# itshawi/data-accelerator

Measured on AMD Instinct MI355X. Metric: events/sec (node) + p99 latency, SimulatedData IoT Flow, higher is better.
Workload: dtype fp64/int64 columns (no reduced precision)

## Files before the change

### dxa/ops/csrc/json_parse.hip

```cpp
#include "dxa_common.h"
#include <type_traits>
#include "decimal_dd.h"
#include "dxa_ts.h"

namespace {

enum : int32_t {
  FT_STRUCT = 0, FT_BOOL = 1, FT_LONG = 2, FT_DOUBLE = 3, FT_STRING = 4, FT_RAW = 5,
  FT_TIMESTAMP = 6, FT_INT = 7, FT_DATE = 8, FT_DECIMAL = 9,
  FT_SKIP = 10,
};

struct ParseArgs {
  uint8_t* buf;
  const int64_t* offs;
  int64_t n;
  const uint64_t* lut_keys;
  const int32_t* lut_node;
  int32_t lut_cap;
  const int32_t* node_type;
  const int32_t* val_slot;
  const int32_t* len_slot;
  int32_t nnodes;
  int64_t* vals;
  int32_t* lens;
  uint8_t* valid;
  uint8_t* row_ok;
  const int32_t* first_child;
  const int32_t* next_sib;
  const int32_t* key_word;
  const int32_t* key_len;
  const uint64_t* key_words;
  int32_t nkey_words;
  const int64_t* ends;
  int64_t* vals2;
  int32_t* lens2;
  uint8_t* valid2;
  int32_t nkv, nkl, nkn;
  const int32_t* zslots;
  int32_t nz;
};

#define G1 __attribute__((address_space(1)))
typedef G1 uint8_t gu8;
struct GArgs {
  gu8* buf;
  const G1 int64_t* offs;
  int64_t n;
  const G1 uint64_t* lut_keys;
  const G1 int32_t* lut_node;
  int32_t lut_cap;
  const G1 int32_t* node_type;
  const G1 int32_t* val_slot;
  const G1 int32_t* len_slot;
  int32_t nnodes;
  G1 int64_t* vals;
  G1 int32_t* lens;
  gu8* valid;
  gu8* row_ok;
  const G1 int32_t* first_child;
  const G1 int32_t* next_sib;
  const G1 int32_t* key_word;
  const G1 int32_t* key_len;
  const G1 uint64_t* key_words;
  int32_t nkey_words;
  const G1 int64_t* ends;
  G1 int64_t* vals2;
  G1 int32_t* lens2;
  gu8* valid2;
  int32_t nkv, nkl, nkn;
  const G1 int32_t* zslots;
  int32_t nz;
  __device__ __forceinline__ G1 int64_t* vrow(int v) const {
    return v < nkv ? vals + (int64_t)v * n : vals2 + (int64_t)(v - nkv) * n;
  }
  __device__ __forceinline__ G1 int32_t* lrow(int l) const {
    return l < nkl ? lens + (int64_t)l * n : lens2 + (int64_t)(l - nkl) * n;
  }
  __device__ __forceinline__ gu8* drow(int k) const {
    return k < nkn ? valid + (int64_t)k * n : valid2 + (int64_t)(k - nkn) * n;
  }
};

__device__ __forceinline__ GArgs to_global(const ParseArgs& p) {
  GArgs g;
  g.buf = (gu8*)p.buf;
  g.offs = (const G1 int64_t*)p.offs;
  g.n = p.n;
  g.lut_keys = (const G1 uint64_t*)p.lut_keys;
  g.lut_node = (const G1 int32_t*)p.lut_node;
  g.lut_cap = p.lut_cap;
  g.node_type = (const G1 int32_t*)p.node_type;
  g.val_slot = (const G1 int32_t*)p.val_slot;
  g.len_slot = (const G1 int32_t*)p.len_slot;
  g.nnodes = p.nnodes;
  g.vals = (G1 int64_t*)p.vals;
  g.lens = (G1 int32_t*)p.lens;
  g.valid = (gu8*)p.valid;
  g.row_ok = (gu8*)p.row_ok;
  g.first_child = (const G1 int32_t*)p.first_child;
  g.next_sib = (const G1 int32_t*)p.next_sib;
  g.key_word = (const G1 int32_t*)p.key_word;
  g.key_len = (const G1 int32_t*)p.key_len;
  g.key_words = (const G1 uint64_t*)p.key_words;
  g.nkey_words = p.nkey_words;
  g.ends = (const G1 int64_t*)p.ends;
  g.vals2 = (G1 int64_t*)p.vals2;
  g.lens2 = (G1 int32_t*)p.lens2;
  g.valid2 = (gu8*)p.valid2;
  g.nkv = p.nkv;
  g.nkl = p.nkl;
  g.nkn = p.nkn;
  g.zslots = (const G1 int32_t*)p.zslots;
  g.nz = p.nz;
  return g;
}

__constant__ uint64_t kPow10i[9] = {1ull, 10ull, 100ull, 1000ull, 10000ull, 100000ull, 1000000ull, 10000000ull,
                                    100000000ull};
__constant__ double kPow10[23] = {1e0,  1e1,  1e2,  1e3,  1e4,  1e5,  1e6,  1e7,  1e8,  1e9,  1e10, 1e11,
                                  1e12, 1e13, 1e14, 1e15, 1e16, 1e17, 1e18, 1e19, 1e20, 1e21, 1e22};


#define G3 __attribute__((address_space(3)))
template <bool LDS>
struct Tables {
  typedef typename std::conditional<LDS, const G3 int32_t*, const G1 int32_t*>::type I32P;
  typedef typename std::conditional<LDS, const G3 uint64_t*, const G1 uint64_t*>::type U64P;
  I32P node_type, val_slot, len_slot, first_child, next_sib, key_word, key_len, lut_node;
  U64P key_words, lut_keys;
  int32_t lut_cap;
};

__host__ __device__ inline int64_t tables_lds_bytes(int32_t nnodes, int32_t nkw, int32_t lut_cap) {
  return (int64_t)nkw * 8 + (int64_t)lut_cap * 8 + (int64_t)(8 * nnodes + lut_cap) * 4;
}

template <bool LDS>
__device__ __forceinline__ Tables<LDS> load_tables(const GArgs& a);

template <>
__device__ __forceinline__ Tables<false> load_tables<false>(const GArgs& a) {
  Tables<false> t;
  t.node_type = a.node_type; t.val_slot = a.val_slot; t.len_slot = a.len_slot;
  t.first_child = a.first_child; t.next_sib = a.next_sib; t.key_word = a.key_word; t.key_len = a.key_len;
  t.lut_node = a.lut_node; t.key_words = a.key_words; t.lut_keys = a.lut_keys; t.lut_cap = a.lut_cap;
  return t;
}

extern __shared__ uint64_t dyn_lds[];

template <>
__device__ __forceinline__ Tables<true> load_tables<true>(const GArgs& a) {
  G3 uint64_t* u64 = (G3 uint64_t*)dyn_lds;
  G3 uint64_t* kw = u64;
  G3 uint64_t* lk = u64 + a.nkey_words;
  G3 int32_t* i32 = (G3 int32_t*)(lk + a.lut_cap);
  const int nn = a.nnodes;
  G3 int32_t* arr[7] = {i32, i32 + nn, i32 + 2 * nn, i32 + 3 * nn, i32 + 4 * nn, i32 + 5 * nn, i32 + 6 * nn};
  G3 int32_t* ln = i32 + 8 * nn;
  for (int i = threadIdx.x; i < a.nkey_words; i += blockDim.x) kw[i] = a.key_words[i];
  for (int i = threadIdx.x; i < a.lut_cap; i += blockDim.x) { lk[i] = a.lut_keys[i]; ln[i] = a.lut_node[i]; }
  for (int i = threadIdx.x; i < nn; i += blockDim.x) {
    arr[0][i] = a.node_type[i]; arr[1][i] = a.val_slot[i]; arr[2][i] = a.len_slot[i];
    arr[3][i] = a.first_child[i]; arr[4][i] = a.next_sib[i]; arr[5][i] = a.key_word[i]; arr[6][i] = a.key_len[i];
  }
  __syncthreads();
// ... 539 lines not shown
  } b{rd};
  auto num = [&](int64_t& i, int digits, int& v) -> bool {
    v = 0;
    for (int k = 0; k < digits; ++k) {
      if (i >= e || !is_digit(b[i])) return false;
      v = v * 10 + (b[i] - '0');
      ++i;
    }
    return true;
  };
  int64_t i = s;
  int y, mo, d, hh = 0, mi = 0, ss = 0;
  if (!num(i, 4, y) || i >= e || b[i] != '-') return false;
  ++i;
  if (!num(i, 2, mo) || i >= e || b[i] != '-') return false;
  ++i;
  if (!num(i, 2, d)) return false;
  int64_t frac_us = 0;
  int64_t tz_us = 0;
  if (i < e && (b[i] == 'T' || b[i] == ' ')) {
    ++i;
    if (!num(i, 2, hh) || i >= e || b[i] != ':') return false;
    ++i;
    if (!num(i, 2, mi)) return false;
    if (i < e && b[i] == ':') { ++i; if (!num(i, 2, ss)) return false; }
    if (i < e && b[i] == '.') {
      ++i;
      int64_t scale = 100000;
      while (i < e && is_digit(b[i])) { frac_us += (b[i] - '0') * scale; scale /= 10; ++i; }
    }
    if (i < e && b[i] == 'Z') ++i;
    else if (i < e && (b[i] == '+' || b[i] == '-')) {
      const bool neg = b[i] == '-';
      ++i;
      int th, tm = 0;
      if (!num(i, 2, th)) return false;
      if (i < e && b[i] == ':') ++i;
      if (i < e) { if (!num(i, 2, tm)) return false; }
      tz_us = ((int64_t)th * 3600 + tm * 60) * 1000000ll;
      if (neg) tz_us = -tz_us;
    }
  } else if (!date_only_ok) {
    return false;
  }
  if (i != e) return false;
  if (mo < 1 || mo > 12 || d < 1 || d > 31 || hh > 23 || mi > 59 || ss > 60) return false;
  const int64_t days = dxa::days_from_civil(y, (unsigned)mo, (unsigned)d);
  out = ((days * 86400 + hh * 3600 + mi * 60 + ss) * 1000000ll) + frac_us - tz_us;
  return true;
}

constexpr uint32_t kTopUp = 32;
typedef int16_t StackT;
template <bool LDS>
__global__ __launch_bounds__(256) __attribute__((amdgpu_waves_per_eu(5))) void json_parse_kernel(ParseArgs pa) {
  const GArgs a = to_global(pa);
  const Tables<LDS> tb = load_tables<LDS>(a);
  const int64_t row = (int64_t)blockIdx.x * blockDim.x + threadIdx.x;
  if (row >= a.n) return;
  for (int j = 0; j < a.nz; ++j) {
    a.vrow(a.zslots[2 * j])[row] = 0;
    a.lrow(a.zslots[2 * j + 1])[row] = 0;
  }
  const int64_t n = a.n;
  Reader r;
  r.buf = a.buf;
  r.p = a.offs[row];
  r.end = a.ends ? a.ends[row] : a.offs[row + 1];
  r.wb = -256;
  r.lim = a.offs[n] + 16;
  __shared__ uint32_t s_win[17][256];
  r.win = (G3U32*)&s_win[0][threadIdx.x];

  __shared__ StackT s_stack[kMaxDepth][256];
  __shared__ StackT s_expect[kMaxDepth][256];
  StackT* stack_ = &s_stack[0][threadIdx.x];
  StackT* expect_ = &s_expect[0][threadIdx.x];
#define stack(i) stack_[(i) * 256]
#define expect(i) expect_[(i) * 256]
  int depth = 0;
  bool ok = false;
  bool comma = false;
  int store_node = -1;
  __shared__ uint64_t s_seen[256];
  s_seen[threadIdx.x] = 0;

  if (r.ws_cur() != '{') goto done;
  ++r.p;
  stack(0) = 0;
  expect(0) = tb.first_child[0];
  depth = 1;
  a.drow(0)[row] = 1;
  uint32_t nextc;
  while (true) {
    r.top_up(kTopUp);
    nextc = 256u;
    uint32_t c;
    int node;
    if (comma) {
      const int ex = expect(depth - 1);
      uint32_t nx = 256u;
      if (ex >= 0 && quote_key_colon(r, r.p, r.end, tb.key_words + tb.key_word[ex], tb.key_len[ex], nx)) {
        comma = false;
        store_node = -1;
        node = ex;
        expect(depth - 1) = tb.next_sib[node];
        c = (nx == 256u || nx == ' ' || nx == '\n' || nx == '\r' || nx == '\t') ? r.ws_cur() : nx;
        goto have_value;
      }
    }
    c = r.ws_cur();
    if (c == '}') {
// ... 135 lines not shown
      }
      if (c == 't' || c == 'f') {
        const int64_t s = r.p;
        const bool v = (c == 't');
        if (!take_literal(r, c)) break;
        if (t == FT_BOOL) {
          a.vrow(vs)[row] = v ? 1 : 0;
          a.drow(node)[row] = 1;
        } else if (t == FT_STRING) {
          a.vrow(vs)[row] = s;
          a.lrow(ls)[row] = v ? 4 : 5;
          a.drow(node)[row] = 1;
        }
        goto after_value;
      }
      if (c == 'n') {
        if (!take_literal(r, c)) break;
        goto after_value;
      }
      break;
    }
  skip_any: {
      const int64_t s0 = r.p;
      if (c == '-' || is_digit(c)) {
        if (!skip_number(r, c, nextc)) break;
      } else if (c == '"') {
        int64_t s, e;
        bool esc;
        if (!scan_string(r, s, e, esc, nextc)) break;
      } else if (!skip_value(r)) {
        break;
      }
      if (store_node >= 0) {
        a.vrow(tb.val_slot[store_node])[row] = s0;
        a.lrow(tb.len_slot[store_node])[row] = (int32_t)(r.p - s0);
        a.drow(store_node)[row] = 1;
      }
    }
  after_value:
    c = (nextc == 256u || nextc == ' ' || nextc == '\n' || nextc == '\r' || nextc == '\t') ? r.ws_cur() : nextc;
    if (c == ',') { ++r.p; comma = true; continue; }
    if (c == '}') continue;
    break;
  }
  if (ok) {
    r.skip_ws();
    ok = r.p >= r.end;
  }
done:
  a.row_ok[row] = ok ? 1 : 0;
  if (!ok) {
    for (int k = 0; k < a.nnodes; ++k) a.drow(k)[row] = 0;
  }
#undef stack
#undef expect
}

__global__ __launch_bounds__(256) void null_count_kernel(const uint8_t* __restrict__ valid, int64_t n,
                                                         unsigned long long* __restrict__ nulls) {
  const int k = blockIdx.y;
  const int64_t r0 = ((int64_t)blockIdx.x * blockDim.x + threadIdx.x) * 8;
  unsigned long long cnt = 0;
  if (r0 < n) {
    const int32_t avail = n - r0 < 8 ? (int32_t)(n - r0) : 8;
    const uint8_t* p = valid + (int64_t)k * n + r0;
    const uintptr_t x = reinterpret_cast<uintptr_t>(p);
    const int m = (int)(x & 7);
    const uint64_t* q = reinterpret_cast<const uint64_t*>(x - m);
    uint64_t v = q[0] >> (8 * m);
    if (m && 8 - m < avail) v |= q[1] << (64 - 8 * m);
    if (avail < 8) v &= (1ull << (8 * avail)) - 1;
    cnt = (unsigned long long)(avail - __popcll(v & 0x0101010101010101ull));
  }
#pragma unroll
  for (int o = 32; o >= 1; o >>= 1) cnt += __shfl_xor(cnt, o);
  if ((threadIdx.x & 63) == 0 && cnt) atomicAdd(&nulls[k], cnt);
}

__device__ __forceinline__ uint64_t nl_bytes(uint64_t x) {
  const uint64_t t = x ^ 0x0a0a0a0a0a0a0a0aull;
  const uint64_t y = ((t & 0x7f7f7f7f7f7f7f7full) + 0x7f7f7f7f7f7f7f7full) | t;
  return ~y & 0x8080808080808080ull;
}

__device__ __forceinline__ void nl_masks(const uint8_t* buf, int64_t p, int64_t end, uint64_t& m0, uint64_t& m1) {
  m0 = m1 = 0;
  if (p >= end) return;
  const uint4 v = *reinterpret_cast<const uint4*>(buf + p);
  m0 = nl_bytes(((uint64_t)v.y << 32) | v.x);
  m1 = nl_bytes(((uint64_t)v.w << 32) | v.z);
  const int64_t rem = end - p;
  if (rem < 16) {
    if (rem <= 8) { m1 = 0; if (rem < 8) m0 &= (1ull << (8 * rem)) - 1; }
    else m1 &= (1ull << (8 * (rem - 8))) - 1;
  }
}

__device__ __forceinline__ uint32_t nl_pack8(uint64_t m) { return (uint32_t)(((m >> 7) * 0x0102040810204080ull) >> 56); }

__global__ __launch_bounds__(256) void count_newlines_kernel(const uint8_t* __restrict__ buf, int64_t len,
                                                             int64_t seg, int64_t nseg,
                                                             int64_t* __restrict__ counts,
                                                             uint16_t* __restrict__ bits) {
  const int lane = threadIdx.x & 63;
  const int64_t s = (int64_t)blockIdx.x * 4 + (threadIdx.x >> 6);
  if (s >= nseg) return;
  const int64_t beg = s * seg;
  const int64_t end = beg + seg < len ? beg + seg : len;
// ... 14 lines not shown
                                                                  int64_t* __restrict__ pos, int64_t cap,
                                                                  int64_t delta) {
  const int lane = threadIdx.x & 63;
  const int64_t s = (int64_t)blockIdx.x * 4 + (threadIdx.x >> 6);
  if (s >= nseg) return;
  const int64_t beg = s * seg;
  const int64_t end = beg + seg < len ? beg + seg : len;
  int64_t k = base[s];
  for (int64_t it = beg; it < end; it += 1024) {
    const int64_t p = it + lane * 16;
    uint32_t m = p < end ? bits[p >> 4] : 0u;
    const uint32_t c = __popc(m);
    uint32_t incl = c;
    for (int o = 1; o < 64; o <<= 1) {
      const uint32_t v = __shfl_up(incl, o, 64);
      if (lane >= o) incl += v;
    }
    int64_t q = k + (incl - c);
    while (m) { const int j = __builtin_ctz(m); if (q < cap) pos[q] = p + j + delta; ++q; m &= m - 1; }
    k += __shfl(incl, 63, 64);
  }
}

__global__ void zero_bytes_kernel(uint8_t* __restrict__ p, int64_t nbytes) {
  const uintptr_t a = reinterpret_cast<uintptr_t>(p);
  const int64_t head = (int64_t)((16 - (a & 15)) & 15) < nbytes ? (int64_t)((16 - (a & 15)) & 15) : nbytes;
  const int64_t body = (nbytes - head) / 16;
  const int64_t tid = (int64_t)blockIdx.x * blockDim.x + threadIdx.x;
  const int64_t stride = (int64_t)gridDim.x * blockDim.x;
  uint4* q = reinterpret_cast<uint4*>(p + head);
  for (int64_t i = tid; i < body; i += stride) q[i] = make_uint4(0, 0, 0, 0);
  const int64_t tail0 = head + body * 16;
  if (tid < head) p[tid] = 0;
  if (tid < nbytes - tail0) p[tail0 + tid] = 0;
}

hipError_t zero_bytes(uint8_t* p, int64_t nbytes, hipStream_t s) {
  if (nbytes <= 0) return hipSuccess;
  const int64_t body = nbytes / 16 + 1;
  const int64_t blocks = (body + 255) / 256 < 4096 ? (body + 255) / 256 : 4096;
  hipLaunchKernelGGL(zero_bytes_kernel, dim3((unsigned)blocks), dim3(256), 0, s, p, nbytes);
  return hipGetLastError();
}

}

DXA_API int dxa_json_parse(uint8_t* buf, const int64_t* offs, int64_t n, const uint64_t* lut_keys,
                           const int32_t* lut_node, int32_t lut_cap, const int32_t* node_type,
                           const int32_t* val_slot, const int32_t* len_slot, int32_t nnodes, int64_t* vals,
                           int32_t* lens, uint8_t* valid, uint8_t* row_ok, const int32_t* first_child,
                           const int32_t* next_sib, const int32_t* key_word, const int32_t* key_len,
                           const uint64_t* key_words, int32_t nkey_words, const int64_t* ends, int64_t* vals2,
                           int32_t* lens2, uint8_t* valid2, int32_t nkv, int32_t nkl, int32_t nkn,
                           const int32_t* zslots, int32_t nz, void* stream) {
  if (n <= 0) return 0;
  if (nnodes >= 32767) return (int)hipErrorInvalidValue;
  if (nkn < 1 || nkn > nnodes) return (int)hipErrorInvalidValue;
  ParseArgs a{buf, offs, n, lut_keys, lut_node, lut_cap, node_type, val_slot, len_slot, nnodes, vals, lens,
              valid, row_ok, first_child, next_sib, key_word, key_len, key_words, nkey_words, ends, vals2, lens2,
              valid2, nkv, nkl, nkn, zslots, nz};
  hipStream_t s = (hipStream_t)stream;
  hipError_t e = zero_bytes(valid, (int64_t)nkn * n, s);
  if (e != hipSuccess) return (int)e;
  if (nnodes > nkn) {
    e = zero_bytes(valid2, (int64_t)(nnodes - nkn) * n, s);
    if (e != hipSuccess) return (int)e;
  }
  const int block = 256;
  const int64_t grid = (n + block - 1) / block;
  const int64_t tab_bytes = tables_lds_bytes(nnodes, nkey_words, lut_cap);
  if (tab_bytes <= 24 * 1024)
    hipLaunchKernelGGL(json_parse_kernel<true>, dim3((unsigned)grid), dim3(block), (size_t)tab_bytes, s, a);
  else
    hipLaunchKernelGGL(json_parse_kernel<false>, dim3((unsigned)grid), dim3(block), 0, s, a);
  return (int)hipGetLastError();
}

DXA_API int dxa_null_counts(const uint8_t* valid, int64_t n, int32_t nnodes, unsigned long long* nulls, void* stream) {
  hipStream_t s = (hipStream_t)stream;
  hipError_t e = hipMemsetAsync(nulls, 0, sizeof(unsigned long long) * (size_t)nnodes, s);
  if (e != hipSuccess) return (int)e;
  if (n <= 0 || nnodes <= 0) return 0;
  hipLaunchKernelGGL(null_count_kernel, dim3((unsigned)((n + 2047) / 2048), (unsigned)nnodes), dim3(256), 0, s, valid, n,
                     nulls);
  return (int)hipGetLastError();
}

DXA_API int dxa_count_newlines(const uint8_t* buf, int64_t len, int64_t seg, int64_t* counts, uint16_t* bits,
                               void* stream) {
  if (len <= 0) return 0;
  if (((uintptr_t)buf & 15) || (seg & 1023)) return (int)hipErrorInvalidValue;
  const int64_t nseg = (len + seg - 1) / seg;
  hipLaunchKernelGGL(count_newlines_kernel, dim3((unsigned)((nseg + 3) / 4)), dim3(256), 0, (hipStream_t)stream, buf,
                     len, seg, nseg, counts, bits);
  return (int)hipGetLastError();
}

DXA_API int dxa_write_newlines_bits(const uint16_t* bits, int64_t len, int64_t seg, const int64_t* base, int64_t* pos,
                                    int64_t cap, int64_t delta, void* stream) {
  if (len <= 0) return 0;
  if (seg & 1023) return (int)hipErrorInvalidValue;
  const int64_t nseg = (len + seg - 1) / seg;
  hipLaunchKernelGGL(write_newlines_bits_kernel, dim3((unsigned)((nseg + 3) / 4)), dim3(256), 0, (hipStream_t)stream,
                     bits, len, seg, nseg, base, pos, cap, delta);
  return (int)hipGetLastError();
}
```

### dxa/ops/jsonparse.py

```python
from __future__ import annotations

import json
import math
from dataclasses import dataclass
from typing import Dict, List, Optional, Sequence, Set, Tuple

import numpy as np
import torch

from . import native as N
from decimal import Decimal as _Decimal

from ..engine.decimal import from_text as decimal_from_text, is_decimal, quantize as decimal_quantize
from ..engine.types import ArrayType, MapType, StructField, StructType

FT = {"struct": 0, "boolean": 1, "long": 2, "double": 3, "float": 3, "decimal": 3, "string": 4, "raw": 5,
      "timestamp": 6, "int": 7, "date": 8, "decimal_exact": 9,
      "short": 7, "byte": 7}
FT_DECIMAL = 9
FT_SKIP = 10

FNV_BASIS = 0xcbf29ce484222325
FNV_PRIME = 0x100000001b3
M64 = (1 << 64) - 1
GOLD = 0x9E3779B97F4A7C15


def _fnv1a(b: bytes) -> int:
    h = FNV_BASIS
    for c in b:
        h = ((h ^ c) * FNV_PRIME) & M64
    return h


def _fmix64(x: int) -> int:
    x ^= x >> 33
    x = (x * 0xff51afd7ed558ccd) & M64
    x ^= x >> 33
    x = (x * 0xc4ceb9fe1a85ec53) & M64
    x ^= x >> 33
    return x


def _to_i64(x: int) -> int:
    return x - (1 << 64) if x >= (1 << 63) else x


@dataclass
class Node:
    path: Tuple[str, ...]
    parent: int
    name: str
    dtype: object
    code: int
    val_slot: int = -1
    len_slot: int = -1
    dropped: bool = False
    shadow: int = 0
    shadow_of: int = -1
    order: int = 0


class ParsePlan:

    def __init__(self, schema: StructType, keep: Optional[Set[Tuple[str, ...]]] = None, skip_unread: bool = False,
                 ts_shadow: Optional[Set[Tuple[str, ...]]] = None):
        self.schema = schema
        self.nodes: List[Node] = [Node((), -1, "", schema, 0)]
        self.keep = keep
        self.skip_unread = skip_unread
        self._build(schema, 0, ())
        for path in sorted(ts_shadow or ()):
            low = tuple(p.lower() for p in path)
            for idx, nd in enumerate(self.nodes[1:], start=1):
                if tuple(p.lower() for p in nd.path) == low and nd.code == FT["string"] and not nd.shadow:
                    self.nodes.append(Node(nd.path + ("#ts",), -1, "", "timestamp", FT["timestamp"], shadow_of=idx))
                    nd.shadow = len(self.nodes) - 1
                    break
        self._kept_first()
        nv = nl = 0
        for nd in self.nodes[1:]:
            if nd.code not in (0, FT_SKIP):
                nd.val_slot = nv
                nv += 1
                if nd.code in (4, 5, FT_DECIMAL):
                    nd.len_slot = nl
                    nl += 1
        self.nval, self.nlen = nv, nl
        self.nkv = sum(1 for nd in self.nodes[:self.nkn] if nd.val_slot >= 0)
        self.nkl = sum(1 for nd in self.nodes[:self.nkn] if nd.len_slot >= 0)
        self.max_depth = max((len(nd.path) for nd in self.nodes if nd.code == 0), default=0)
        cap = 1 << max(4, math.ceil(math.log2(max(2, 2 * len(self.nodes)))))
        keys = [0] * cap
        node_of = [-1] * cap
        for idx, nd in enumerate(self.nodes[1:], start=1):
            if nd.shadow_of >= 0:
                continue
            k = _fmix64(_fnv1a(nd.name.encode("utf-8")) ^ (((nd.parent + 1) * GOLD) & M64))
            if k == 0:
                k = 1
            s = k & (cap - 1)
            while keys[s] != 0:
                s = (s + 1) & (cap - 1)
            keys[s] = k
            node_of[s] = idx
        self.lut_keys = [_to_i64(k) for k in keys]
        self.lut_node = node_of
        self.cap = cap
        nn = len(self.nodes)
        self.first_child = [-1] * nn
        self.next_sib = [-1] * nn
        last = {}
        for idx in sorted(range(1, nn), key=lambda i: self.nodes[i].order):
            nd = self.nodes[idx]
            if nd.shadow_of >= 0:
                continue
            if nd.parent in last:
                self.next_sib[last[nd.parent]] = idx
            else:
                self.first_child[nd.parent] = idx
            last[nd.parent] = idx
        words, self.key_word, self.key_len = [], [0] * nn, [0] * nn
        for idx, nd in enumerate(self.nodes):
            b = nd.name.encode("utf-8")
            self.key_word[idx], self.key_len[idx] = len(words), len(b)
            b += b"\0" * (-len(b) % 8)
            words += [int.from_bytes(b[i:i + 8], "little") for i in range(0, len(b), 8)]
        self.key_words = [_to_i64(w) for w in words] or [0]
        self._dev: Dict[str, Tuple[torch.Tensor, ...]] = {}

    def _kept_first(self):
        for i, nd in enumerate(self.nodes):
            nd.order = i
        kept = lambda nd: not nd.dropped and nd.code != FT_SKIP
        new = [0] + [i for i in range(1, len(self.nodes)) if kept(self.nodes[i])] + \
            [i for i in range(1, len(self.nodes)) if not kept(self.nodes[i])]
        remap = {old: k for k, old in enumerate(new)}
        nodes = [self.nodes[i] for i in new]
        for nd in nodes:
            if nd.parent >= 0:
                nd.parent = remap[nd.parent]
            if nd.shadow:
                nd.shadow = remap[nd.shadow]
            if nd.shadow_of >= 0:
                nd.shadow_of = remap[nd.shadow_of]
        self.nodes = nodes
        self.nkn = 1 + sum(1 for nd in nodes[1:] if kept(nd))

    def _wanted(self, path) -> bool:
        if self.keep is None:
            return True
        return any(k[:len(path)] == path or path[:len(k)] == k for k in self.keep)

    def _build(self, st: StructType, parent: int, prefix, dropped: bool = False):
        for f in st.fields:
            path = prefix + (f.name,)
            drop = dropped or not self._wanted(path)
            if drop and self.skip_unread:
                self.nodes.append(Node(path, parent, f.name, f.dtype, FT_SKIP))
                if isinstance(f.dtype, StructType):
                    self._build_skipped(f.dtype, len(self.nodes) - 1, path)
                continue
            if isinstance(f.dtype, StructType):
                self.nodes.append(Node(path, parent, f.name, f.dtype, 0, dropped=drop))
                self._build(f.dtype, len(self.nodes) - 1, path, drop)
            elif isinstance(f.dtype, (MapType, ArrayType)):
                self.nodes.append(Node(path, parent, f.name, f.dtype, FT["raw"], dropped=drop))
            else:
                code = FT_DECIMAL if is_decimal(f.dtype) else FT.get(f.dtype, FT["string"])
                self.nodes.append(Node(path, parent, f.name, f.dtype, code, dropped=drop))

    def _build_skipped(self, st: StructType, parent: int, prefix):
        for f in st.fields:
            self.nodes.append(Node(prefix + (f.name,), parent, f.name, f.dtype, FT_SKIP))
            if isinstance(f.dtype, StructType):
                self._build_skipped(f.dtype, len(self.nodes) - 1, prefix + (f.name,))

    def string_slot_pairs(self, device) -> Optional[torch.Tensor]:
        key = ("zslots", str(device))
        if key not in self._dev:
            pairs = [(nd.val_slot, nd.len_slot) for nd in self.nodes[1:self.nkn] if nd.code in (4, 5, FT_DECIMAL)]
            self._dev[key] = torch.tensor([v for p in pairs for v in p], dtype=torch.int32, device=device) \
# ... 31 lines not shown
    if torch.device(device).type != "cpu":
        buf, o = buf.to(device, non_blocking=True), o.to(device, non_blocking=True)
    return buf, o


def frame_lines_gpu(buf: torch.Tensor, length: int, expected: Optional[int] = None,
                    mismatches: Optional[list] = None) -> torch.Tensor:
    seg = 1 << 16
    nseg = (length + seg - 1) // seg
    dev = buf.device
    if buf.data_ptr() % 16:
        buf = buf.clone()
    counts = torch.empty(max(nseg, 1), dtype=torch.int64, device=dev)
    bits = torch.empty(max((length + 15) // 16, 1), dtype=torch.int16, device=dev)
    st = N.stream_handle(dev)
    if length:
        N.call("dxa_count_newlines", N.ptr(buf), length, seg, N.ptr(counts), N.ptr(bits), st)
    counts = counts[:nseg]
    base = torch.cumsum(counts, 0) - counts
    total = expected if expected is not None else (int(counts.sum().item()) if nseg else 0)
    if expected is not None:
        offs = torch.empty(total + 1, dtype=torch.int64, device=dev)
        offs[:1].zero_()
        if length:
            N.call("dxa_write_newlines_bits", N.ptr(bits), length, seg, N.ptr(base), N.ptr(offs[1:]), total, 1, st)
            found = counts.sum()
            offs[1:].masked_fill_(torch.arange(1, total + 1, device=dev) > found, length)
            if mismatches is not None:
                mismatches.append(found != total)
        else:
            offs[1:].fill_(0)
            if mismatches is not None:
                mismatches.append(torch.full((), bool(total != 0), dtype=torch.bool, device=dev))
        return offs
    pos = torch.empty(max(total, 1), dtype=torch.int64, device=dev)
    if length:
        N.call("dxa_write_newlines_bits", N.ptr(bits), length, seg, N.ptr(base), N.ptr(pos), total, 0, st)
    pos = pos[:total]
    ends = torch.cat([pos + 1, N.h2d([length], torch.int64, dev)])
    starts = torch.cat([torch.zeros(1, dtype=torch.int64, device=dev), pos + 1])
    keep = (ends - starts) > 1
    starts, ends = starts[keep], ends[keep]
    return torch.cat([starts, ends[-1:]]) if starts.numel() else torch.zeros(1, dtype=torch.int64, device=dev)


def check_framing(mismatches: list):
    if mismatches:
        bad = int(torch.stack([m.reshape(()) for m in mismatches]).sum().item())
        mismatches.clear()
        if bad:
            raise ValueError(f"{bad} framed batch(es) held a different record count than their producer declared")


def parse(buf: torch.Tensor, offs: torch.Tensor, plan: ParsePlan, ends: Optional[torch.Tensor] = None):
    return parse_async(buf, offs, plan, ends).result()


class PendingParse:

    def __init__(self, done=None, plan=None, arena=None, parts=None, n=0, counts=None, event=None, stream=None):
        self._done = done
        self.plan, self.arena, self.parts, self.n = plan, arena, parts, n
        self.counts, self.event, self.stream = counts, event, stream

    def result(self):
        if self._done is None:
            if self.event is not None:
                self.event.synchronize()
            nulls = self.counts.tolist() if self.counts is not None else [1] * len(self.plan.nodes)
            vals, lens, valid, row_ok = self.parts
            if self.stream is not None and self.arena is not None:
                cur = torch.cuda.current_stream(self.arena.device)
                if cur != self.stream:
                    for t in (vals, lens, valid, row_ok, self.arena):
                        t.record_stream(cur)
            ps = getattr(self, "pane_stats", None)
            if ps is not None:
                from ..engine.windows import register_pane_stats
                for (slot, _row), st in zip(ps[0], ps[1].tolist()):
                    register_pane_stats(vals[slot].data_ptr(), self.n, st, self.arena.data_ptr())
            self._done = (_assemble(self.plan, self.arena, vals, lens, valid, self.n, nulls), row_ok)
            self.parts = self.arena = self.counts = self.event = self.stream = None
        return self._done


def parse_async(buf: torch.Tensor, offs: torch.Tensor, plan: ParsePlan,
                ends: Optional[torch.Tensor] = None) -> PendingParse:
    n = int(offs.shape[0]) - 1
    if buf.device.type == "cuda" and plan.max_depth < GPU_MAX_DEPTH:
        return _parse_gpu_async(buf, offs, n, plan, ends)
    if buf.device.type == "cuda":
        col, ok = _parse_cpu(buf.cpu(), offs.cpu(), n, plan, None if ends is None else ends.cpu())
        return PendingParse(done=(col.to(buf.device), ok.to(buf.device)))
    return PendingParse(done=_parse_cpu(buf, offs, n, plan, ends))


GPU_MAX_DEPTH = 8


def _parse_gpu(buf, offs, n, plan: ParsePlan, ends=None):
    return _parse_gpu_async(buf, offs, n, plan, ends).result()


def _parse_gpu_async(buf, offs, n, plan: ParsePlan, ends=None) -> PendingParse:
    lut_k, lut_n, types, vslot, lslot, fchild, nsib, kword, klen, kwords = plan.device_tables(buf.device)
    nn = len(plan.nodes)
    m = max(n, 1)
    vals = torch.empty((max(1, plan.nkv), m), dtype=torch.int64, device=buf.device)
    lens = torch.empty((max(1, plan.nkl), m), dtype=torch.int32, device=buf.device)
    valid = torch.empty((plan.nkn, m), dtype=torch.uint8, device=buf.device)
    vals2 = torch.empty((max(1, plan.nval - plan.nkv), m), dtype=torch.int64, device=buf.device)
    lens2 = torch.empty((max(1, plan.nlen - plan.nkl), m), dtype=torch.int32, device=buf.device)
    valid2 = torch.empty((max(1, nn - plan.nkn), m), dtype=torch.uint8, device=buf.device)
    row_ok = torch.empty(max(n, 1), dtype=torch.uint8, device=buf.device)
    zs = plan.string_slot_pairs(buf.device)
    counts = event = pane_stats = None
    if n:
        st = N.stream_handle(buf.device)
        N.call("dxa_json_parse", N.ptr(buf), N.ptr(offs), n, N.ptr(lut_k), N.ptr(lut_n), plan.cap, N.ptr(types),
               N.ptr(vslot), N.ptr(lslot), nn, N.ptr(vals), N.ptr(lens), N.ptr(valid), N.ptr(row_ok),
               N.ptr(fchild), N.ptr(nsib), N.ptr(kword), N.ptr(klen), N.ptr(kwords), int(kwords.numel()),
               None if ends is None else N.ptr(ends), N.ptr(vals2), N.ptr(lens2), N.ptr(valid2), plan.nkv,
               plan.nkl, plan.nkn, N.ptr(zs), 0 if zs is None else zs.numel() // 2, st)
        nk = plan.nkn
        cnt = torch.empty(nk, dtype=torch.int64, device=buf.device)
        N.call("dxa_null_counts", N.ptr(valid), n, nk, N.ptr(cnt), st)
        counts = torch.empty(nk, dtype=torch.int64, pin_memory=True)
        counts.copy_(cnt, non_blocking=True)
        shadows = [(plan.nodes[i].val_slot, i) for i in range(1, plan.nkn) if plan.nodes[i].shadow_of >= 0]
        if shadows:
            from ..engine.windows import queue_pane_stats
            pst = queue_pane_stats(vals, valid, lens[:plan.nkl] if plan.nkl else lens[:0], n, shadows)
            pane_stats = (shadows, torch.empty(pst.shape, dtype=torch.int64, pin_memory=True))
            pane_stats[1].copy_(pst, non_blocking=True)
        event = torch.cuda.Event()
        event.record(torch.cuda.current_stream(buf.device))
    parts = (vals[:, :n], lens[:, :n], valid[:, :n].view(torch.bool), row_ok[:n].view(torch.bool))
    pp = PendingParse(plan=plan, arena=buf, parts=parts, n=n, counts=counts, event=event,
                      stream=torch.cuda.current_stream(buf.device))
    pp.pane_stats = pane_stats
    return pp


def _assemble(plan: ParsePlan, arena, vals, lens, valid, n, nulls=None):
    from ..engine.column import PrimColumn, StrColumn, JsonColumn, StructColumn
    device = arena.device
    cols: Dict[int, object] = {}
    for idx in range(len(plan.nodes) - 1, 0, -1):
        nd = plan.nodes[idx]
        if nd.code == FT_SKIP or nd.dropped or nd.shadow_of >= 0:
            continue
        v = valid[idx] if (nulls is None or nulls[idx]) else None
        if nd.code == 0:
            kids = [(plan.nodes[j].name, cols[j]) for j in range(len(plan.nodes))
                    if plan.nodes[j].parent == idx and j in cols]
            cols[idx] = StructColumn([k for k, _ in kids], [c for _, c in kids], n, v, False, None, device)
            continue
        raw = vals[nd.val_slot]
        if nd.code == FT["string"]:
            cols[idx] = StrColumn(arena, raw, lens[nd.len_slot], v)
            if nd.shadow:
                sh = nd.shadow
                cols[idx]._parsed_ts = PrimColumn("timestamp", vals[plan.nodes[sh].val_slot],
                                                  valid[sh] if (nulls is None or nulls[sh]) else None)
        elif nd.code == FT["raw"]:
            cols[idx] = JsonColumn(arena, raw, lens[nd.len_slot], v, nd.dtype)
        elif nd.code == FT_DECIMAL:
            cols[idx] = decimal_from_text(StrColumn(arena, raw, lens[nd.len_slot], v), nd.dtype, trim=False)
        elif nd.code == FT["double"]:
            cols[idx] = PrimColumn(nd.dtype if nd.dtype in ("double", "float", "decimal") else "double",
                                   raw.view(torch.float64), v)
        elif nd.code == FT["boolean"]:
            cols[idx] = PrimColumn("boolean", raw != 0, v)
        elif nd.dtype in ("short", "byte"):
            from ..engine.types import INT_RANGE
            lo, hi = INT_RANGE[nd.dtype]
            inr = (raw >= lo) & (raw <= hi)
            cols[idx] = PrimColumn(nd.dtype, raw, inr if v is None else v & inr)
        else:
            cols[idx] = PrimColumn(nd.dtype, raw, v)
    kids = [(plan.nodes[j].name, cols[j]) for j in range(1, len(plan.nodes)) if plan.nodes[j].parent == 0 and j in cols]
    root_valid = valid[0] if (nulls is None or nulls[0]) else None
    return StructColumn([k for k, _ in kids], [c for _, c in kids], n, root_valid, False, None, device)


def _iso_to_us(s: str) -> Optional[int]:
    import re
    import datetime as dt
    m = re.match(r"^(\d{4})-(\d{2})-(\d{2})(?:[T ](\d{2}):(\d{2})(?::(\d{2}))?(?:\.(\d+))?(Z|[+-]\d{2}:?(?:\d{2})?)?)?$",
                 s)
    if not m:
        return None
    y, mo, d = int(m.group(1)), int(m.group(2)), int(m.group(3))
# ... 133 lines not shown
```

### dxa/ops/native.py

```python
from __future__ import annotations

import ctypes
import os
import threading
from pathlib import Path

import torch

_LIB = None
_LOCK = threading.Lock()
_HERE = Path(__file__).resolve().parent
LIB_PATH = Path(os.environ.get("DXA_NATIVE_LIB") or (_HERE / "_native" / "libdxa_kernels.so"))

c_i64 = ctypes.c_int64
c_i32 = ctypes.c_int32
c_p = ctypes.c_void_p

_SIGS = {
    "dxa_byte_map": [c_p, c_p, c_i64, c_p, c_p],
    "dxa_lz4_block_sizes": [c_p, c_p, c_p, c_p, c_i64, c_i64, c_p, c_p, c_p],
    "dxa_lz4_decode": [c_p, c_p, c_p, c_p, c_p, c_p, c_i64, c_i64, c_p, c_p, c_p],
    "dxa_memcpy_h2d_async": [c_p, c_p, c_i64, c_p],
    "dxa_copy_sdma": [c_p, c_p, c_i64],
    "dxa_lz4_decode_into": [c_p, c_p, c_p, c_p, c_p, c_p, c_i64, c_p, c_p, c_p, c_p],
    "dxa_inflate_into": [c_p, c_p, c_p, c_p, c_p, c_p, c_i64, c_p, c_p, c_p, c_p],
    "dxa_snappy_decode_into": [c_p, c_p, c_p, c_p, c_p, c_p, c_i64, c_p, c_p, c_p, c_p],
    "dxa_zstd_decode_into": [c_p, c_p, c_p, c_p, c_p, c_p, c_i64, c_p, c_p, c_p, c_p],
    "dxa_zstd_decode_prof": [c_p, c_p, c_p, c_p, c_p, c_p, c_i64, c_p, c_p, c_p, c_p, c_p],
    "dxa_kafka_records": [c_p, c_i64] + [c_p] * 14,
    "dxa_kafka_crc": [c_p, c_i64, c_p, c_p, c_p, c_p, c_p],
    "dxa_csv_tokenize": [c_p, c_p, c_i64, c_i32, c_i32, c_i32, c_i32, c_p, c_p, c_p, c_p, c_p],
    "dxa_spark_hash_fixed": [c_p, c_i32, c_p, c_i64, c_p, c_p],
    "dxa_spark_hash_str": [c_p, c_p, c_p, c_p, c_i64, c_p, c_p],
    "dxa_serialize_rows": [c_i32, c_p, c_i32, c_i32, c_i32, c_p, c_p, c_p, c_p, c_p],
    "dxa_java_double_dev": [c_p, c_i64, c_p, c_p, c_p],
    "dxa_java_double_hostcheck": [c_p, c_i64, c_p, c_p],
    "dxa_json_parse": [c_p, c_p, c_i64, c_p, c_p, c_i32, c_p, c_p, c_p, c_i32, c_p, c_p, c_p, c_p,
                       c_p, c_p, c_p, c_p, c_p, c_i32, c_p, c_p, c_p, c_p, c_i32, c_i32, c_i32, c_p, c_i32,
                       c_p],
    "dxa_count_newlines": [c_p, c_i64, c_i64, c_p, c_p, c_p],
    "dxa_write_newlines_bits": [c_p, c_i64, c_i64, c_p, c_p, c_i64, c_i64, c_p],
    "dxa_null_counts": [c_p, c_i64, c_i32, c_p, c_p],
    "dxa_hash_i64": [c_p, c_p, c_i64, c_p, ctypes.c_int, c_p],
    "dxa_hash_f64": [c_p, c_p, c_i64, c_p, ctypes.c_int, c_p],
    "dxa_hash_str": [c_p, c_p, c_p, c_p, c_i64, c_p, ctypes.c_int, c_p],
    "dxa_table_insert": [c_p, c_i64, c_p, c_i64, c_p, c_p],
    "dxa_group_ids": [c_p, c_i64, c_p, c_i64, c_p, c_p, c_p, c_p, c_p],
    "dxa_verify_i64": [c_p, c_p, c_p, c_p, c_i64, c_p, c_p],
    "dxa_verify_f64": [c_p, c_p, c_p, c_p, c_i64, c_p, c_p],
    "dxa_verify_str": [c_p, c_p, c_p, c_p, c_p, c_p, c_i64, c_p, c_p],
    "dxa_aggregate": [c_p, c_p, c_p, c_i64, c_i32, c_i32, c_i32, c_p, c_p],
    "dxa_aggregate_multi": [c_p, c_i64, c_i32, c_i32, c_p, c_i32, c_p, c_p, c_p],
    "dxa_aggregate_finish": [c_p, c_i32, c_i32, c_i32, c_p, c_p, c_p, c_p],
    "dxa_partial_finish_size": [],
    "dxa_partial_finish": [c_p, c_p],
    "dxa_group_renumber": [c_p, c_i64, c_p, c_i32, c_p, c_p, c_p],
    "dxa_group_build": [c_p, c_i64, c_p, c_i64, c_p, c_p, c_p, c_p, c_p],
    "dxa_group_build_init": [c_p, c_i64, c_p, c_i64, c_p, c_p, c_p, c_p, c_p],
    "dxa_slot_count": [c_p, c_i64, c_p, c_p],
    "dxa_slot_scatter": [c_p, c_i64, c_p, c_p, c_p, c_p],
    "dxa_probe_count": [c_p, c_p, c_i64, c_p, c_i64, c_p, c_p, c_p, ctypes.c_int, c_p],
    "dxa_probe_write": [c_p, c_i64, c_p, c_p, c_p, c_p, c_p, c_p, ctypes.c_int, c_p],
    "dxa_str_cmp_lit": [c_p, c_p, c_p, c_i64, c_p, c_i32, c_i32, c_p, c_p],
    "dxa_str_eq_col": [c_p, c_p, c_p, c_p, c_p, c_p, c_i64, c_p, c_p],
    "dxa_str_cmp_col": [c_p, c_p, c_p, c_p, c_p, c_p, c_i64, c_i32, c_p, c_p],
    "dxa_str_gather": [c_p, c_p, c_p, c_i64, c_p, c_p, c_p],
    "dxa_str_gather_parts": [c_p, c_i32, c_p],
    "dxa_str_split_count": [c_p, c_p, c_p, c_i64, c_p, c_i32, c_p, c_p],
    "dxa_ts_format": [c_p, c_i64, c_p, c_i32, c_p, c_i32, c_p, c_p],
    "dxa_str_like": [c_p, c_p, c_p, c_i64, c_p, c_i32, c_p, c_p],
    "dxa_str_rlike": [c_p, c_p, c_p, c_i64, c_p, c_i32, c_i32, c_i32, c_p, c_p],
    "dxa_str_regex": [c_p, c_p, c_p, c_i64, c_p, c_i32, c_p, c_i32, c_i32, c_i32, c_p, c_i32, c_p, c_p, c_p, c_p, c_p,
                      c_p, c_p],
    "dxa_gzip_chunks": [c_p, c_i64, c_i32, c_p, c_p, c_i32, c_p, c_p],
    "dxa_gzip_pack": [c_p, c_i32, c_p, c_p, c_i64, c_p, c_p],
    "dxa_str_digest": [c_p, c_p, c_p, c_i64, c_i32, c_p, c_p],
    "dxa_str_crc32": [c_p, c_p, c_p, c_i64, c_p, c_p],
    "dxa_str_encode": [c_p, c_p, c_p, c_i64, c_i32, c_p, c_p, c_p],
    "dxa_f64_str_len": [c_p, c_p, c_i64, c_p, c_p],
    "dxa_f64_str_write": [c_p, c_p, c_i64, c_p, c_p, c_p],
    "dxa_str_to_num": [c_p, c_p, c_p, c_p, c_i64, c_i32, c_p, c_p, c_p],
    "dxa_concat_ws_len": [c_p, c_i32, c_i64, c_i32, c_p, c_p],
    "dxa_concat_ws_write": [c_p, c_i32, c_i64, c_p, c_i32, c_p, c_p, c_p],
    "dxa_str_substr": [c_p, c_p, c_p, c_i64, c_p, c_i64, c_p, c_i64, c_p, c_p, c_p],
    "dxa_str_trim": [c_p, c_p, c_p, c_i64, c_i32, c_p, c_p, c_p],
    "dxa_str_numchars": [c_p, c_p, c_p, c_i64, c_p, c_p],
    "dxa_str_locate": [c_p, c_p, c_p, c_i64, c_p, c_i32, c_i64, c_p, c_p],
    "dxa_str_replace_len": [c_p, c_p, c_p, c_i64, c_p, c_i32, c_i32, c_p, c_p],
    "dxa_str_replace_write": [c_p, c_p, c_p, c_i64, c_p, c_i32, c_p, c_i32, c_p, c_p, c_p],
    "dxa_str_split_write": [c_p, c_p, c_p, c_i64, c_p, c_i32, c_i32, c_p, c_p, c_p],
    "dxa_str_part_size": [],
    "dxa_concat_len": [c_p, c_i32, c_i64, c_p, c_p, c_p],
# ... 121 lines not shown
```

Before: 252.4 million.

## Add schema-specialized uniform JSON parse with compacted fallback rows

Compiles the parse plan into a linear program of expected byte patterns and typed leaf ops, and runs a new kernel that matches each record against this fixed schema order without hash lookups or stack tracking. Rows that deviate are collected by ballot-based atomic compaction into a fallback list. The generic kernel then reprocesses only those rows with a capped, grid-strided launch. This aims to remove the divergent general-purpose parse cost for uniformly shaped IoT records. The cost is an extra kernel launch and a small counter memset, with extra work when many rows deviate from the expected key order.

```diff
diff --git a/dxa/ops/csrc/json_parse.hip b/dxa/ops/csrc/json_parse.hip
--- a/dxa/ops/csrc/json_parse.hip
+++ b/dxa/ops/csrc/json_parse.hip
@@ -39,6 +39,10 @@
   int32_t nkv, nkl, nkn;
   const int32_t* zslots;
   int32_t nz;
+  const uint64_t* prog;
+  int32_t nops;
+  int32_t* fb_rows;
+  int32_t* fb_count;
 };
 
 #define G1 __attribute__((address_space(1)))
@@ -71,6 +75,8 @@
   int32_t nkv, nkl, nkn;
   const G1 int32_t* zslots;
   int32_t nz;
+  G1 int32_t* fb_rows;
+  G1 int32_t* fb_count;
   __device__ __forceinline__ G1 int64_t* vrow(int v) const {
     return v < nkv ? vals + (int64_t)v * n : vals2 + (int64_t)(v - nkv) * n;
   }
@@ -113,6 +119,8 @@
   g.nkn = p.nkn;
   g.zslots = (const G1 int32_t*)p.zslots;
   g.nz = p.nz;
+  g.fb_rows = (G1 int32_t*)p.fb_rows;
+  g.fb_count = (G1 int32_t*)p.fb_count;
   return g;
 }
 
@@ -758,12 +766,23 @@
 
 constexpr uint32_t kTopUp = 32;
 typedef int16_t StackT;
-template <bool LDS>
+#ifndef DXA_PARSE_FALLBACK_BLOCKS
+#define DXA_PARSE_FALLBACK_BLOCKS 1280
+#endif
+constexpr int64_t kFallbackBlocks = DXA_PARSE_FALLBACK_BLOCKS;
+template <bool LDS, bool IDX>
 __global__ __launch_bounds__(256) __attribute__((amdgpu_waves_per_eu(5))) void json_parse_kernel(ParseArgs pa) {
   const GArgs a = to_global(pa);
+  const int64_t nrows = IDX ? (int64_t)a.fb_count[0] : a.n;
+  if (IDX && (int64_t)blockIdx.x * blockDim.x >= nrows) return;
   const Tables<LDS> tb = load_tables<LDS>(a);
-  const int64_t row = (int64_t)blockIdx.x * blockDim.x + threadIdx.x;
-  if (row >= a.n) return;
+  for (int64_t i0 = (int64_t)blockIdx.x * blockDim.x;; i0 += (int64_t)gridDim.x * blockDim.x) {
+  int64_t row = i0 + threadIdx.x;
+  if (row >= nrows) return;
+  if (IDX) {
+    row = a.fb_rows[row];
+    for (int k = 0; k < a.nnodes; ++k) a.drow(k)[row] = 0;
+  }
   for (int j = 0; j < a.nz; ++j) {
     a.vrow(a.zslots[2 * j])[row] = 0;
     a.lrow(a.zslots[2 * j + 1])[row] = 0;
@@ -1005,8 +1024,122 @@
   if (!ok) {
     for (int k = 0; k < a.nnodes; ++k) a.drow(k)[row] = 0;
   }
+  if (!IDX) return;
+  }
 #undef stack
 #undef expect
+}
+
+constexpr int kOpWords = 8;
+constexpr int kOpPattern = 3;
+#ifndef DXA_PARSE_UNIFORM_WAVES
+#define DXA_PARSE_UNIFORM_WAVES 5
+#endif
+__global__ __launch_bounds__(256) __attribute__((amdgpu_waves_per_eu(DXA_PARSE_UNIFORM_WAVES)))
+void json_parse_uniform_kernel(ParseArgs pa) {
+  const GArgs a = to_global(pa);
+  typedef const __attribute__((address_space(4))) uint64_t* ProgP;
+  const ProgP prog = (ProgP)pa.prog;
+  const int nops = pa.nops;
+  const int64_t n = a.n;
+  const int64_t row_ = (int64_t)blockIdx.x * blockDim.x + threadIdx.x;
+  const bool in = row_ < n;
+  const int64_t row = in ? row_ : n - 1;
+  Reader r;
+  r.buf = a.buf;
+  r.p = a.offs[row];
+  r.end = a.ends ? a.ends[row] : a.offs[row + 1];
+  r.wb = -256;
+  r.lim = a.offs[n] + 16;
+  __shared__ uint32_t s_win[18][256];
+  r.win = (G3U32*)&s_win[0][threadIdx.x];
+  bool live = in;
+  for (int pc = 0; pc < nops; ++pc) {
+    if (__builtin_amdgcn_ballot_w64(live) == 0) break;
+    const ProgP op = prog + pc * kOpWords;
+    const uint64_t w0 = op[0];
+    const int kind = (int)(w0 & 0xff);
+    const int plen = (int)((w0 >> 8) & 0xff);
+    if (!live) continue;
+    r.top_up(kTopUp);
+    if (r.p + plen > r.end) { live = false; continue; }
+    bool m = true;
+    for (int j = 0; 8 * j < plen; ++j) {
+      const int nb = plen - 8 * j;
+      const uint64_t mask = nb >= 8 ? ~0ull : ((1ull << (8 * nb)) - 1);
+      m &= ((r.load8(r.p + 8 * j) ^ op[kOpPattern + j]) & mask) == 0;
+    }
+    if (!m) { live = false; continue; }
+    r.p += plen;
+    const uint64_t w2 = op[2];
+    const int node = (int)(w2 & 0xffff);
+    if (kind == 0) {
+      if (node != 0xffff) a.drow(node)[row] = 1;
+      continue;
+    }
+    const uint64_t w1 = op[1];
+    const int vs = (int)(uint32_t)w1;
+    const uint32_t c = r.cur();
+    if (kind == FT_STRING || kind == FT_TIMESTAMP || kind == FT_DATE) {
+      int64_t s, e;
+      bool esc;
+      uint32_t after;
+      if (c != '"' || !scan_string(r, s, e, esc, after) || esc) { live = false; continue; }
+      if (kind == FT_STRING) {
+        a.vrow(vs)[row] = s;
+        a.lrow((int)(w1 >> 32))[row] = (int32_t)(e - s);
+        a.drow(node)[row] = 1;
+        const int sh = (int)((w2 >> 16) & 0xffff);
+        if (sh != 0xffff) {
+          int64_t us;
+          if (dxa::string_to_ts((const uint8_t*)(r.buf + s), (int32_t)(e - s), us)) {
+            a.vrow((int)(w2 >> 32))[row] = us;
+            a.drow(sh)[row] = 1;
+          }
+        }
+      } else {
+        int64_t us;
+        if (parse_iso_ts(r, s, e, us, true)) {
+          a.vrow(vs)[row] = (kind == FT_DATE) ? (us >= 0 ? us / 86400000000ll
+                                                         : -((-us + 86399999999ll) / 86400000000ll))
+                                              : us;
+          a.drow(node)[row] = 1;
+        }
+      }
+    } else if (kind == FT_BOOL) {
+      if ((c != 't' && c != 'f') || !take_literal(r, c)) { live = false; continue; }
+      a.vrow(vs)[row] = c == 't' ? 1 : 0;
+      a.drow(node)[row] = 1;
+    } else {
+      bool is_int, of;
+      int64_t iv = 0;
+      double dv = 0.0;
+      uint32_t term;
+      if ((c != '-' && !is_digit(c)) || !scan_number(r, c, is_int, of, iv, dv, term)) { live = false; continue; }
+      if (kind == FT_DOUBLE) {
+        a.vrow(vs)[row] = __double_as_longlong(dv);
+        a.drow(node)[row] = 1;
+      } else if (is_int && !of && (kind == FT_LONG || (iv >= -2147483648ll && iv <= 2147483647ll))) {
+        a.vrow(vs)[row] = iv;
+        a.drow(node)[row] = 1;
+      }
+    }
+  }
+  if (live) {
+    r.skip_ws();
+    live = r.p >= r.end;
+  }
+  if (live) a.row_ok[row] = 1;
+  const bool dev = in && !live;
+  const uint64_t bm = __builtin_amdgcn_ballot_w64(dev);
+  if (bm) {
+    const int lane = (int)(threadIdx.x & 63);
+    const int leader = __builtin_ctzll(bm);
+    int32_t base = 0;
+    if (lane == leader) base = atomicAdd((int32_t*)pa.fb_count, (int32_t)__popcll(bm));
+    base = __shfl(base, leader, 64);
+    if (dev) a.fb_rows[base + __popcll(bm & ((1ull << lane) - 1))] = (int32_t)row;
+  }
 }
 
 __global__ __launch_bounds__(256) void null_count_kernel(const uint8_t* __restrict__ valid, int64_t n,
@@ -1127,15 +1260,18 @@
                            const int32_t* next_sib, const int32_t* key_word, const int32_t* key_len,
                            const uint64_t* key_words, int32_t nkey_words, const int64_t* ends, int64_t* vals2,
                            int32_t* lens2, uint8_t* valid2, int32_t nkv, int32_t nkl, int32_t nkn,
-                           const int32_t* zslots, int32_t nz, void* stream) {
+                           const int32_t* zslots, int32_t nz, const uint64_t* prog, int32_t nops,
+                           int32_t* fb_rows, int32_t* fb_count, void* stream) {
   if (n <= 0) return 0;
   if (nnodes >= 32767) return (int)hipErrorInvalidValue;
   if (nkn < 1 || nkn > nnodes) return (int)hipErrorInvalidValue;
   ParseArgs a{buf, offs, n, lut_keys, lut_node, lut_cap, node_type, val_slot, len_slot, nnodes, vals, lens,
               valid, row_ok, first_child, next_sib, key_word, key_len, key_words, nkey_words, ends, vals2, lens2,
-              valid2, nkv, nkl, nkn, zslots, nz};
+              valid2, nkv, nkl, nkn, zslots, nz, prog, nops, fb_rows, fb_count};
   hipStream_t s = (hipStream_t)stream;
-  hipError_t e = zero_bytes(valid, (int64_t)nkn * n, s);
+  const int64_t vz = (int64_t)nkn * n, vz4 = (vz + 3) & ~3ll;
+  const bool counter_behind = prog && (uint8_t*)fb_count == valid + vz4;
+  hipError_t e = zero_bytes(valid, counter_behind ? vz4 + 4 : vz, s);
   if (e != hipSuccess) return (int)e;
   if (nnodes > nkn) {
     e = zero_bytes(valid2, (int64_t)(nnodes - nkn) * n, s);
@@ -1144,10 +1280,26 @@
   const int block = 256;
   const int64_t grid = (n + block - 1) / block;
   const int64_t tab_bytes = tables_lds_bytes(nnodes, nkey_words, lut_cap);
+  if (prog) {
+    if (nops <= 0 || !fb_rows || !fb_count || n > 0x7fffffffll) return (int)hipErrorInvalidValue;
+    if (!counter_behind) {
+      e = hipMemsetAsync(fb_count, 0, sizeof(int32_t), s);
+      if (e != hipSuccess) return (int)e;
+    }
+    hipLaunchKernelGGL(json_parse_uniform_kernel, dim3((unsigned)grid), dim3(block), 0, s, a);
+    e = hipGetLastError();
+    if (e != hipSuccess) return (int)e;
+    const int64_t fgrid = grid < kFallbackBlocks ? grid : kFallbackBlocks;
+    if (tab_bytes <= 24 * 1024)
+      hipLaunchKernelGGL((json_parse_kernel<true, true>), dim3((unsigned)fgrid), dim3(block), (size_t)tab_bytes, s, a);
+    else
+      hipLaunchKernelGGL((json_parse_kernel<false, true>), dim3((unsigned)fgrid), dim3(block), 0, s, a);
+    return (int)hipGetLastError();
+  }
   if (tab_bytes <= 24 * 1024)
-    hipLaunchKernelGGL(json_parse_kernel<true>, dim3((unsigned)grid), dim3(block), (size_t)tab_bytes, s, a);
+    hipLaunchKernelGGL((json_parse_kernel<true, false>), dim3((unsigned)grid), dim3(block), (size_t)tab_bytes, s, a);
   else
-    hipLaunchKernelGGL(json_parse_kernel<false>, dim3((unsigned)grid), dim3(block), 0, s, a);
+    hipLaunchKernelGGL((json_parse_kernel<false, false>), dim3((unsigned)grid), dim3(block), 0, s, a);
   return (int)hipGetLastError();
 }
 
diff --git a/dxa/ops/jsonparse.py b/dxa/ops/jsonparse.py
--- a/dxa/ops/jsonparse.py
+++ b/dxa/ops/jsonparse.py
@@ -59,6 +59,24 @@
     shadow: int = 0
     shadow_of: int = -1
     order: int = 0
+
+
+PROG_PUNCT = 0
+PROG_LEAF_CODES = (FT["boolean"], FT["long"], FT["double"], FT["string"], FT["timestamp"], FT["int"], FT["date"])
+PROG_OP_WORDS = 8
+PROG_PATTERN_WORDS = 5
+PROG_NONE = 0xFFFF
+
+
+@dataclass
+class ProgOp:
+    kind: int
+    pattern: bytes
+    node: int = PROG_NONE
+    val_slot: int = 0
+    len_slot: int = 0
+    shadow_node: int = PROG_NONE
+    shadow_slot: int = 0
 
 
 class ParsePlan:
@@ -127,7 +145,60 @@
             b += b"\0" * (-len(b) % 8)
             words += [int.from_bytes(b[i:i + 8], "little") for i in range(0, len(b), 8)]
         self.key_words = [_to_i64(w) for w in words] or [0]
+        self.program: Optional[List[ProgOp]] = self._build_program()
         self._dev: Dict[str, Tuple[torch.Tensor, ...]] = {}
+
+    def _build_program(self) -> Optional[List["ProgOp"]]:
+        if self.max_depth >= GPU_MAX_DEPTH or len(self.nodes) >= PROG_NONE:
+            return None
+        ops = [ProgOp(PROG_PUNCT, b"{", 0)]
+
+        def walk(parent: int) -> bool:
+            child, first = self.first_child[parent], True
+            while child >= 0:
+                nd = self.nodes[child]
+                key = nd.name.encode("utf-8")
+                if nd.code not in PROG_LEAF_CODES and nd.code != 0:
+                    return False
+                if any(c < 0x20 or c in b'"\\' for c in key):
+                    return False
+                pat = (b"" if first else b",") + b'"' + key + b'":'
+                if nd.code == 0:
+                    ops.append(ProgOp(PROG_PUNCT, pat + b"{", child))
+                    if not walk(child):
+                        return False
+                    ops.append(ProgOp(PROG_PUNCT, b"}"))
+                else:
+                    sh = nd.shadow
+                    ops.append(ProgOp(nd.code, pat, child, nd.val_slot, max(nd.len_slot, 0), sh or PROG_NONE,
+                                      self.nodes[sh].val_slot if sh else 0))
+                child, first = self.next_sib[child], False
+            return True
+
+        if not walk(0):
+            return None
+        ops.append(ProgOp(PROG_PUNCT, b"}"))
+        if any(len(op.pattern) > 8 * PROG_PATTERN_WORDS for op in ops) or self.nval >= (1 << 31):
+            return None
+        return ops
+
+    def program_words(self) -> Optional[List[int]]:
+        if self.program is None:
+            return None
+        words = []
+        for op in self.program:
+            pat = op.pattern + b"\0" * (8 * PROG_PATTERN_WORDS - len(op.pattern))
+            words += [op.kind | len(op.pattern) << 8, op.val_slot | op.len_slot << 32,
+                      op.node | op.shadow_node << 16 | op.shadow_slot << 32]
+            words += [int.from_bytes(pat[i:i + 8], "little") for i in range(0, len(pat), 8)]
+        return [_to_i64(w) for w in words]
+
+    def device_program(self, device) -> Optional[torch.Tensor]:
+        key = ("program", str(device))
+        if key not in self._dev:
+            w = self.program_words()
+            self._dev[key] = None if w is None else torch.tensor(w, dtype=torch.int64, device=device)
+        return self._dev[key]
 
     def _kept_first(self):
         for i, nd in enumerate(self.nodes):
@@ -265,14 +336,16 @@
             raise ValueError(f"{bad} framed batch(es) held a different record count than their producer declared")
 
 
-def parse(buf: torch.Tensor, offs: torch.Tensor, plan: ParsePlan, ends: Optional[torch.Tensor] = None):
-    return parse_async(buf, offs, plan, ends).result()
+def parse(buf: torch.Tensor, offs: torch.Tensor, plan: ParsePlan, ends: Optional[torch.Tensor] = None,
+          fast: bool = True):
+    return parse_async(buf, offs, plan, ends, fast=fast).result()
 
 
 class PendingParse:
 
     def __init__(self, done=None, plan=None, arena=None, parts=None, n=0, counts=None, event=None, stream=None):
         self._done = done
+        self.fallback_rows: Optional[torch.Tensor] = None
         self.plan, self.arena, self.parts, self.n = plan, arena, parts, n
         self.counts, self.event, self.stream = counts, event, stream
 
@@ -298,10 +371,10 @@
 
 
 def parse_async(buf: torch.Tensor, offs: torch.Tensor, plan: ParsePlan,
-                ends: Optional[torch.Tensor] = None) -> PendingParse:
+                ends: Optional[torch.Tensor] = None, fast: bool = True) -> PendingParse:
     n = int(offs.shape[0]) - 1
     if buf.device.type == "cuda" and plan.max_depth < GPU_MAX_DEPTH:
-        return _parse_gpu_async(buf, offs, n, plan, ends)
+        return _parse_gpu_async(buf, offs, n, plan, ends, fast)
     if buf.device.type == "cuda":
         col, ok = _parse_cpu(buf.cpu(), offs.cpu(), n, plan, None if ends is None else ends.cpu())
         return PendingParse(done=(col.to(buf.device), ok.to(buf.device)))
@@ -315,26 +388,34 @@
     return _parse_gpu_async(buf, offs, n, plan, ends).result()
 
 
-def _parse_gpu_async(buf, offs, n, plan: ParsePlan, ends=None) -> PendingParse:
+def _parse_gpu_async(buf, offs, n, plan: ParsePlan, ends=None, fast: bool = True,
+                     keep_dropped: bool = False) -> PendingParse:
     lut_k, lut_n, types, vslot, lslot, fchild, nsib, kword, klen, kwords = plan.device_tables(buf.device)
     nn = len(plan.nodes)
     m = max(n, 1)
     vals = torch.empty((max(1, plan.nkv), m), dtype=torch.int64, device=buf.device)
     lens = torch.empty((max(1, plan.nkl), m), dtype=torch.int32, device=buf.device)
-    valid = torch.empty((plan.nkn, m), dtype=torch.uint8, device=buf.device)
+    vbytes = plan.nkn * m
+    vflat = torch.empty(((vbytes + 3) & ~3) + 4, dtype=torch.uint8, device=buf.device)
+    valid = vflat[:vbytes].view(plan.nkn, m)
     vals2 = torch.empty((max(1, plan.nval - plan.nkv), m), dtype=torch.int64, device=buf.device)
     lens2 = torch.empty((max(1, plan.nlen - plan.nkl), m), dtype=torch.int32, device=buf.device)
     valid2 = torch.empty((max(1, nn - plan.nkn), m), dtype=torch.uint8, device=buf.device)
     row_ok = torch.empty(max(n, 1), dtype=torch.uint8, device=buf.device)
     zs = plan.string_slot_pairs(buf.device)
-    counts = event = pane_stats = None
+    counts = event = pane_stats = fb_rows = fb_count = None
+    prog = plan.device_program(buf.device) if fast and 0 < n < (1 << 31) else None
+    if prog is not None:
+        fb_rows = torch.empty(n, dtype=torch.int32, device=buf.device)
+        fb_count = vflat[(vbytes + 3) & ~3:].view(torch.int32)
     if n:
         st = N.stream_handle(buf.device)
         N.call("dxa_json_parse", N.ptr(buf), N.ptr(offs), n, N.ptr(lut_k), N.ptr(lut_n), plan.cap, N.ptr(types),
                N.ptr(vslot), N.ptr(lslot), nn, N.ptr(vals), N.ptr(lens), N.ptr(valid), N.ptr(row_ok),
                N.ptr(fchild), N.ptr(nsib), N.ptr(kword), N.ptr(klen), N.ptr(kwords), int(kwords.numel()),
                None if ends is None else N.ptr(ends), N.ptr(vals2), N.ptr(lens2), N.ptr(valid2), plan.nkv,
-               plan.nkl, plan.nkn, N.ptr(zs), 0 if zs is None else zs.numel() // 2, st)
+               plan.nkl, plan.nkn, N.ptr(zs), 0 if zs is None else zs.numel() // 2, N.ptr(prog),
+               0 if prog is None else prog.numel() // PROG_OP_WORDS, N.ptr(fb_rows), N.ptr(fb_count), st)
         nk = plan.nkn
         cnt = torch.empty(nk, dtype=torch.int64, device=buf.device)
         N.call("dxa_null_counts", N.ptr(valid), n, nk, N.ptr(cnt), st)
@@ -352,6 +433,9 @@
     pp = PendingParse(plan=plan, arena=buf, parts=parts, n=n, counts=counts, event=event,
                       stream=torch.cuda.current_stream(buf.device))
     pp.pane_stats = pane_stats
+    pp.fallback_rows = fb_count
+    if keep_dropped:
+        pp.dropped_parts = (vals2[:, :n], lens2[:, :n], valid2[:, :n].view(torch.bool))
     return pp
 
 
diff --git a/dxa/ops/native.py b/dxa/ops/native.py
--- a/dxa/ops/native.py
+++ b/dxa/ops/native.py
@@ -37,7 +37,7 @@
     "dxa_java_double_hostcheck": [c_p, c_i64, c_p, c_p],
     "dxa_json_parse": [c_p, c_p, c_i64, c_p, c_p, c_i32, c_p, c_p, c_p, c_i32, c_p, c_p, c_p, c_p,
                        c_p, c_p, c_p, c_p, c_p, c_i32, c_p, c_p, c_p, c_p, c_i32, c_i32, c_i32, c_p, c_i32,
-                       c_p],
+                       c_p, c_i32, c_p, c_p, c_p],
     "dxa_count_newlines": [c_p, c_i64, c_i64, c_p, c_p, c_p],
     "dxa_write_newlines_bits": [c_p, c_i64, c_i64, c_p, c_p, c_i64, c_i64, c_p],
     "dxa_null_counts": [c_p, c_i64, c_i32, c_p, c_p],
```

Result: no change. 252.1 million (-0.1%).
